# LorenzoNajt/FlipComplexityEmpirical

Measured on AMD Instinct MI355X. Metric: flip proposals/sec (node) 40x40 grid k=2, 1/2/4/8 MI355X; % LDS/HBM roofline, higher is better.
Workload: dtype int8

## Files before the change

### flipcomplexityempirical_amd/csrc/fc_device.h

```cpp
#pragma once
#include <hip/hip_runtime.h>
#include <stdint.h>

#include <type_traits>

#include "fc_internal.h"
#include "fc_philox.h"
#include "fc_ring.h"

namespace fc {
namespace dev {

__device__ __forceinline__ void compiler_fence() { asm volatile("" ::: "memory"); }
__device__ __forceinline__ void wave_sync() { asm volatile("s_waitcnt lgkmcnt(0)" ::: "memory"); }

#ifdef FC_PHASE_PROF
#ifdef FC_PHASE_SYNC
#define FC_STAMP(t)                                                    \
    asm volatile("s_waitcnt vmcnt(0) lgkmcnt(0)" ::: "memory");        \
    const int64_t t = (int64_t)__builtin_amdgcn_s_memtime()
#else
#define FC_STAMP(t) const int64_t t = (int64_t)__builtin_amdgcn_s_memtime()
#endif
#define FC_PROF(i, x) \
    do { if (lane == 0) atomicAdd((unsigned long long *)&prof_acc[i], (unsigned long long)(int64_t)(x)); } while (0)
#else
#define FC_STAMP(t)
#define FC_PROF(i, x)
#endif

__device__ __forceinline__ uint64_t bits_below(int n) { return n >= 64 ? ~0ull : ((1ull << n) - 1ull); }
__device__ __forceinline__ uint64_t lane_range(int lo, int hi) { return bits_below(hi) & ~bits_below(lo); }

__device__ __forceinline__ int rl32(int x, int lane) { return __builtin_amdgcn_readlane(x, lane); }
__device__ __forceinline__ uint32_t rlu(uint32_t x, int lane) { return (uint32_t)__builtin_amdgcn_readlane((int)x, lane); }

__device__ __forceinline__ int64_t rl64(int64_t x, int lane) {
    const uint32_t lo = rlu((uint32_t)x, lane), hi = rlu((uint32_t)((uint64_t)x >> 32), lane);
    return (int64_t)(((uint64_t)hi << 32) | lo);
}
template <typename... T>
__device__ __forceinline__ void wave_sum64_all(T &...x) {
#pragma unroll
    for (int off = 32; off >= 1; off >>= 1) ((x += __shfl_xor((long long)x, off)), ...);
}
__device__ __forceinline__ int64_t wave_sum64(int64_t x) {
    wave_sum64_all(x);
    return x;
}

template <int CTRL>
__device__ __forceinline__ int32_t dpp_pair(int32_t x) {
    return __builtin_amdgcn_update_dpp(x, x, CTRL, 0xf, 0xf, false);
}
constexpr int kQuadSwap1 = 0xB1;
constexpr int kQuadSwap2 = 0x4E;
constexpr int kRowHalfMirror = 0x141;
constexpr int kRowMirror = 0x140;

__device__ __forceinline__ int32_t row0_sum(int32_t x) {
    x += dpp_pair<kQuadSwap1>(x);
    x += dpp_pair<kQuadSwap2>(x);
    x += dpp_pair<kRowHalfMirror>(x);
    x += dpp_pair<kRowMirror>(x);
    return rl32(x, 0);
}
__device__ __forceinline__ int32_t min_lanes32(int32_t x) {
    x = min(x, dpp_pair<kQuadSwap1>(x));
    x = min(x, dpp_pair<kQuadSwap2>(x));
    x = min(x, dpp_pair<kRowHalfMirror>(x));
    x = min(x, dpp_pair<kRowMirror>(x));
    return min(rl32(x, 0), rl32(x, 16));
}

__device__ __forceinline__ int count_below(uint64_t m) {
    return (int)__builtin_amdgcn_mbcnt_hi((uint32_t)(m >> 32), __builtin_amdgcn_mbcnt_lo((uint32_t)m, 0u));
}

template <int CTRL>
__device__ __forceinline__ int dpp_mov(int x) {
    return __builtin_amdgcn_update_dpp(0, x, CTRL, 0xf, 0xf, false);
}

__device__ __forceinline__ int wave_scan_incl(int x) {
    x += dpp_mov<0x111>(x);
    x += dpp_mov<0x112>(x);
    x += dpp_mov<0x114>(x);
    x += dpp_mov<0x118>(x);
    x += __builtin_amdgcn_update_dpp(0, x, 0x142, 0xa, 0xf, false);
    x += __builtin_amdgcn_update_dpp(0, x, 0x143, 0xc, 0xf, false);
    return x;
}

__device__ __forceinline__ int select_bit64(uint64_t x, int r) {
    uint32_t y = (uint32_t)x;
    int pos = 0, c = __popc(y);
    if (r >= c) { r -= c; y = (uint32_t)(x >> 32); pos = 32; }
    c = __popc(y & 0xffffu);
    if (r >= c) { r -= c; y >>= 16; pos += 16; }
    c = __popc(y & 0xffu);
    if (r >= c) { r -= c; y >>= 8; pos += 8; }
    c = __popc(y & 0xfu);
    if (r >= c) { r -= c; y >>= 4; pos += 4; }
    c = __popc(y & 0x3u);
    if (r >= c) { r -= c; y >>= 2; pos += 2; }
    return pos + (r >= (int)(y & 1u) ? 1 : 0);
}

__device__ __forceinline__ int kth_set_bit(uint64_t x, int k) {
    for (int i = 1; i < k; ++i) x &= x - 1;
    return __builtin_ctzll(x);
}

template <int RMAX>
__device__ __forceinline__ int ring_entry(const uint32_t (&ring)[RMAX / 2], int i) {
    return (int)((ring[i >> 1] >> (16 * (i & 1))) & 0xffffu);
}

template <int RMAX>
__device__ __forceinline__ int ring_entry_at(const uint32_t (&ring)[RMAX / 2], uint32_t pos) {
    const uint32_t sel = 0x0c0c0100u + (pos & 3u) * 0x0202u;
    uint32_t e = __builtin_amdgcn_perm(ring[1], ring[0], sel);
#pragma unroll
    for (int k = 1; k < RMAX / 4; ++k) {
        const uint32_t q = __builtin_amdgcn_perm(ring[2 * k + 1], ring[2 * k], sel);
        e = ((pos >> 2) == (uint32_t)k) ? q : e;
    }
    return (int)e;
}

using fc::one_run;
using fc::one_run_flat;

__device__ __forceinline__ int deal_chain(const KParams &p, int lane) {
    int cc = 0;
    if (lane == 0) {
        uint32_t hw, xcc;
        asm volatile("s_getreg_b32 %0, hwreg(HW_REG_HW_ID)" : "=s"(hw));
        asm volatile("s_getreg_b32 %0, hwreg(HW_REG_XCC_ID)" : "=s"(xcc));
        const uint32_t key = ((xcc & 7u) << 12) | ((hw >> 4) & 0xfffu);
        const uint32_t slot = atomicAdd(&p.deal[key], 1u);
        const uint32_t C = (uint32_t)p.n_chains;
        for (uint32_t k = 0; k < 4; ++k) {
            const uint32_t q = (slot + k) & 3u;
            const uint32_t lo = q * C / 4u, hi = (q + 1u) * C / 4u;
            const uint32_t i = atomicAdd(&p.deal[kDealKeys + q], 1u);
            if (lo + i < hi) {
                cc = (int)p.order[lo + i];
                break;
            }
        }
    }
    return __builtin_amdgcn_readfirstlane(__shfl(cc, 0));
}

constexpr int kBfsList = 512;
struct BfsScratch {
    uint32_t *lab;
    uint32_t *mm;
    uint32_t *cm;
// ... 443 lines not shown
```

### flipcomplexityempirical_amd/csrc/fc_flip2.hip

```cpp
#include <hip/hip_runtime.h>

#include <cstdlib>
#include <algorithm>
#include <type_traits>

#include "fc_device.h"
#include "fc_internal.h"
#include "fc_philox.h"
#include "fc_tally.h"

namespace fc {

using namespace dev;

#ifndef FC_PRIO_EVERY_LOG2
#define FC_PRIO_EVERY_LOG2 4
#endif
static_assert(sizeof(KParams) % 8 == 0, "flip2_kernel's second argument sits at sizeof(KParams)");
template <bool FULL>
__device__ __forceinline__ PhiloxKeys batch_keys(PhiloxKeys keys) {
    typedef const unsigned char __attribute__((address_space(4))) *KernArg;
    if constexpr (FULL) {
        KernArg ka = (KernArg)__builtin_amdgcn_kernarg_segment_ptr();
        asm volatile("" : "+s"(ka));
// ... 196 lines not shown
    int prio = 0;
    if (lane == 0) {
        misc[3] = 0;
        misc[4] = (uint64_t)steps_in;
        if (FULL && p.tl_t0) p.tl_t0[c] = steps_in;
        misc[0] = __builtin_amdgcn_s_memrealtime();
        const float eta0 = p.eta ? (float)p.eta[p.eta_parity ^ 1] * (float)p.n_steps * (1.0f / 1024.0f) : 0.0f;
        misc[1] = (uint64_t)__float_as_uint(eta0);
    }
    compiler_fence();
    while (rem > 0) {
        const bool every = ((prio += 4) & (((1 << FC_PRIO_EVERY_LOG2) - 1) << 2)) == 0;
        if (every) cnt_fold();
        if (every && p.prio_nb[0] > 0) {
            const int done = (int)p.n_steps - rem;
            const float eta = __uint_as_float((uint32_t)misc[1]);
            int lv;
            if (eta > 0.0f && done * 16 >= (int)p.n_steps) {
                const float pr = (float)(__builtin_amdgcn_s_memrealtime() - misc[0]) * (float)p.n_steps / ((float)done * eta);
                lv = (pr > p.prio_th[0]) + (pr > p.prio_th[1]) + (pr > p.prio_th[2]);
            } else {
                lv = (nb < p.prio_nb[0]) + (nb < p.prio_nb[1]) + (nb < p.prio_nb[2]);
            }
            if (lv != (prio & 3)) {
                prio = (prio & ~3) | lv;
                switch (lv) {
                    case 0: __builtin_amdgcn_s_setprio(0); break;
                    case 1: __builtin_amdgcn_s_setprio(1); break;
                    case 2: __builtin_amdgcn_s_setprio(2); break;
                    default: __builtin_amdgcn_s_setprio(3); break;
                }
            }
        }
        FC_STAMP(t_a);
        FC_PROF(5, 1);
        if (draw >= draw_cap) {
            stuck = 1;
            break;
        }
        const uint64_t room = draw_cap - draw;
        int nh = 0;
        int gen = 0;
        int rv[kRV];
        auto rv_off = [&](int j, int l) { return BAND ? 64 * j + l : 4 * l + j - (int)(draw & 3u); };
        if constexpr (!BAND) {
            const int s0 = (int)(draw & 3u);
            const int wcap = 64 * NSUB < 4 * kWave - s0 ? 64 * NSUB : 4 * kWave - s0;
            const int win = (uint64_t)wcap < room ? wcap : (int)room;
            const uint64_t q = (draw >> 2) + (uint64_t)lane;
            uint32_t nw[4];
            if (XTRA && p.tape) {
#pragma unroll
                for (int j = 0; j < 4; ++j) {
                    const int off = 4 * lane + j - s0;
                    const bool inr = off >= 0 && off < win;
                    nw[j] = p.tape[((size_t)c * (size_t)p.tape_draws + (inr ? draw + (uint64_t)off : draw)) * 6];
                }
            } else {
                const PhiloxKeys pk = batch_keys<FULL>(keys);
                const Words4 w = philox4x32_10_keys((uint32_t)q, (uint32_t)(q >> 32), chain_gid, 3u, pk);
                nw[0] = w.x0;
                nw[1] = w.x1;
                nw[2] = w.x2;
                nw[3] = w.x3;
            }
            int vdj[4];
            uint32_t okm = 0u, hb = 0u;
#pragma unroll
            for (int j = 0; j < 4; ++j) {
                const int off = 4 * lane + j - s0;
                const uint64_t m = (uint64_t)nw[j] * (uint64_t)(uint32_t)n;
                vdj[j] = (int)(m >> 32);
                const bool ok = (off >= 0) & (off < win) & ((uint32_t)m >= p.lemire_thresh);
                okm |= (uint32_t)ok << j;
                hb |= (uint32_t)(ok & (fcnt[vdj[j]] != 0)) << j;
            }
            const int hc = __popc(hb);
            const int incl = wave_scan_incl(hc);
            const int excl = incl - hc;
            const int tot = rl32(incl, kWave - 1);
            gen = win;
            int lim = 4 * kWave;
            if (tot > 64) {
                const int L = __builtin_ctzll(__ballot(incl >= 64));
                const uint32_t hbL = rlu(hb, L);
                const int k = 64 - rl32(excl, L);
                uint32_t mk = hbL;
                for (int i = 1; i < k; ++i) mk &= mk - 1u;
                const int jj = __builtin_ctz(mk);
                lim = 4 * L + jj - s0 + 1;
                gen = lim;
            }
            uint32_t *const ssink = slot + 256 + lane;
#pragma unroll
            for (int j = 0; j < 4; ++j) {
                const int off = 4 * lane + j - s0;
                const int sp = excl + __popc(hb & ((1u << j) - 1u));
                const bool hit = (hb >> j) & 1u;
                const bool put = hit & (sp < 64);
                *(put ? slot + sp : ssink) = (uint32_t)vdj[j];
                *(put ? slot + 192 + sp : ssink) = (uint32_t)off;
                rv[j] = (((okm >> j) & 1u) & !hit & (off < lim)) ? (vdj[j] | (sp << 16)) : -1;
            }
            nh = tot;
        } else {
            int bpre = 0x7fffffff;
            {
                const int cw = lane < p.words ? (int)__popcll(sb[lane]) : 0;
                const int inc = wave_scan_incl(cw);
                if (lane < p.words) bpre = inc - cw;
            }
#pragma unroll
            for (int r = 0; r < NSUB; ++r) {
                rv[r] = -1;
                if ((r > 0 && nh >= p.hit_stop) || nh >= 64 || (uint64_t)gen >= room) continue;
                const int off = gen + lane;
                const bool inrange = (uint64_t)off < room;
                const uint64_t dr = draw + (uint64_t)off;
                const Words4 w = philox4x32_10((uint32_t)dr, (uint32_t)(dr >> 32), chain_gid, 0u, p.seed_lo, p.seed_hi);
                const uint64_t m = (uint64_t)w.x0 * (uint64_t)nS;
                const int idx = (int)(m >> 32);
                const bool okd = inrange && (uint32_t)m >= thrS;
                int bw = 0, bb = 0;
                for (int st2 = p.band_step0; st2 >= 1; st2 >>= 1) {
                    const int cand = bw + st2;
                    const int pc = __builtin_amdgcn_ds_bpermute(cand << 2, bpre);
                    if (pc <= idx) {
                        bw = cand;
                        bb = pc;
                    }
                }
                const int vd = 64 * bw + select_bit64(sb[bw], idx - bb);
                const bool hitd = okd & (fcnt[vd] != 0);
                const uint64_t hm = __ballot(hitd);
                const int sp = nh + count_below(hm);
                if (hitd && sp < 64) {
                    slot[sp] = (uint32_t)vd;
                    slot[64 + sp] = w.x1;
                    slot[128 + sp] = w.x2;
                    slot[192 + sp] = (uint32_t)off;
                }
                const int cnt = __popcll(hm);
                int used = kWave;
                if (nh + cnt > 64) {
                    used = kth_set_bit(hm, 64 - nh) + 1;
                    gen += used;
                } else {
                    gen = (uint64_t)(gen + 64) < room ? gen + 64 : (int)room;
                }
                rv[r] = (okd & !hitd & (lane < used)) ? (vd | (sp << 16)) : rv[r];
                nh += cnt;
            }
        }
        const int ns = nh < 64 ? nh : 64;
        compiler_fence();
        FC_STAMP(t_b);
        FC_PROF(1, t_b - t_a);

        const bool has = lane < ns;
        const int off_r = (int)slot[192 + lane], v_r = (int)slot[lane];
        int off_l = has ? off_r : gen;
        const uint64_t d = draw + (uint64_t)off_l;
        int v = has ? v_r : 0;
        uint32_t w1, w2;
        if constexpr (BAND) {
            w1 = slot[64 + lane];
            w2 = slot[128 + lane];
// ... 65 lines not shown
        bool rebuild = false;
        const int cut0 = cut, nb0 = nb;
        const int64_t steps0 = FULL ? steps_in + ((int)p.n_steps - rem) : 0;
        const int last_flip0 = last_flip;
        const int a_last0 = FULL && last_flip0 >= 0 ? (int)a[last_flip0] : 0;
        int cut_after = 0, nb_after = 0;
        auto dp_of = [&]() { return av == 0 ? -pv : pv; };
        auto dg_of = [&]() { return (st & LF_GAM) ? (av == 0 ? -1 : 1) : 0; };

        auto reeval = [&](int from, int vfx, uint32_t eqx) {
            FC_STAMP(t_re0);
            compiler_fence();
            if (has && lane >= from) {
                const uint32_t lkl = slot[256 + lane];
                const uint32_t w1r = (!FULL && !BAND) ? w1 : slot[64 + lane], w2r = (!FULL && !BAND) ? w2 : slot[128 + lane];
                if (vfx < 0) {
                    av = a[v];
                    uint32_t i1 = 0;
                    int ad[RMAX];
#pragma unroll
                    for (int i = 0; i < RMAX; ++i) ad[i] = a[cell[i]];
#pragma unroll
                    for (int i = 0; i < RMAX; ++i) asm volatile("" : "+v"(ad[i]));
#pragma unroll
                    for (int i = 0; i < RMAX; ++i) i1 |= (uint32_t)ad[i] << i;
                    inA = av ? i1 : ~i1;
                } else {
                    const bool self = v == vfx;
                    av = self ? 1 - av : av;
                    inA = (self ? ~inA : inA) ^ eqx;
                }
                const uint32_t nbA = inA & nbr;
                tmask = nbr & ~inA;
                nA = __popc(nbA);
                delta = nA - __popc(tmask);
                const uint64_t th = T[delta + RMAX];
                const uint32_t lnk = lkl & 0xffffu, L2 = lkl >> 16;
                const uint32_t fl = (1u << L2) - 1u;
                inA &= fl;
                const uint32_t rot = L2 ? (((inA >> 1) | (inA << (L2 - 1))) & fl) : 0u;
                const uint32_t lk = inA & rot & lnk;
                const bool sl = one_run_flat(nbA, fl & ~lk, fl);
                const uint32_t vlink = (L2 >= 2) ? ((inA & (inA >> (L2 - 1)) & 1u) << (L2 - 1)) : 0u;
                const bool sc = one_run_flat(nbA, fl & ~(lk | vlink), fl);
                const bool ac = mant53(w1r, w2r) < th;
                st = (st & (LF_EXACT | LF_GAM | LF_HAS | LF_FRZ)) | (tmask != 0u ? LF_HIT : 0u) | (ac ? LF_ACC : 0u) |
                     (sl ? LF_SLIN : 0u) | (sc ? LF_SCYC : 0u);
            }
            compiler_fence();
            FC_STAMP(t_re1);
            FC_PROF(16, t_re1 - t_re0);
            FC_PROF(17, 1);
        };

        auto run_bfs = [&](int f) -> bool {
            const uint32_t nbrAf = rlu(inA & nbr, f);
            int my_target = -1, start = -1;
#pragma unroll
            for (int k2 = 0; k2 < RMAX / 2; ++k2) {
                const uint32_t wrd = rlu(rec.ring[k2], f);
                if ((lane >> 1) == k2) my_target = (int)((wrd >> (16 * (lane & 1))) & 0xffffu);
                if (start < 0 && ((nbrAf >> (2 * k2)) & 1u)) start = (int)(wrd & 0xffffu);
                if (start < 0 && ((nbrAf >> (2 * k2 + 1)) & 1u)) start = (int)(wrd >> 16);
            }
            if (!(lane < RMAX && ((nbrAf >> lane) & 1u))) my_target = -1;
            int64_t lv = 0;
            const bool res = wave_bfs_single<RMAX>(G, a, bs, lane, rl32(v, f), rl32(av, f), my_target, start, lv);
            if (lane == 0) {
                atomicAdd((unsigned long long *)&scp->bfs_calls, 1ull);
                atomicAdd((unsigned long long *)&scp->bfs_levels, (unsigned long long)lv);
            }
            return res;
        };

        while (pos < end) {
            FC_PROF(6, 1);
            FC_STAMP(t_it0);
#ifdef FC_PHASE_PROF
            if (first_it) FC_PROF(27, t_it0 - t_c);
            first_it = false;
#endif
            asm volatile("" : "+v"(st), "+v"(inA), "+v"(tmask), "+v"(nbr), "+v"(delta), "+v"(nA), "+v"(av), "+v"(pv),
                         "+v"(v), "+v"(off_l));
            const bool hit = (st & LF_HIT) != 0, acc = (st & LF_ACC) != 0, s_lin = (st & LF_SLIN) != 0,
                       s_cyc = (st & LF_SCYC) != 0, exact = SEARCH ? (st & LF_EXACT) != 0 : true,
                       gam = (st & LF_GAM) != 0, has = (st & LF_HAS) != 0;
            const bool prop = hit & (lane >= pos) & (lane < end);
            const bool bd = SEARCH && (st & ST_BD) != 0, br = SEARCH && (st & ST_BR) != 0, nz = nA != 0;
            const bool okT = bd ? br : (nz & s_lin);
            const bool okN = bd ? br : (nz & ((exact & gam) ? s_cyc : s_lin));
            const bool known = bd | !nz | exact | s_lin;
            const bool ok = ((av ? ng0 : ng1) > 0) ? okT : okN;
            const int pa = av ? pops1 : pops0, pb = av ? pops0 : pops1;
            const bool popok = (pa - pv >= pop_lo) & (pb + pv <= pop_hi);
            bool valid = prop & known & ok & popok;
            bool acc_now = acc;
            bool inv_contig = !ok;
            if constexpr (XTRA) {
                if (p.variant) {
                    const int gm = gam ? 1 : 0;
                    const bool b_ok = ((av ? ng1 : ng0) - gm > 0) && ((av ? ng0 : ng1) + gm > 0);
                    const bool f_ok = !(st & LF_FRZ);
                    auto pass = [&](uint32_t M) {
                        return (!(M & FC_CON_CONTIG) || ok) && (!(M & FC_CON_POP) || popok) &&
                               (!(M & FC_CON_BOUNDARY) || b_ok) && (!(M & FC_CON_FIXED) || f_ok);
                    };
                    valid = prop && known && pass(p.con_valid);
                    inv_contig = (p.con_valid & FC_CON_CONTIG) && !ok;
                    bool au = acc;
                    if (p.accept == FC_ACCEPT_UNIFORM) {
                        au = true;
                    } else if (p.accept == FC_ACCEPT_ANNEAL) {
                        int dnb_l = nA == 0 ? -1 : 0;
#pragma unroll
                        for (int i = 0; i < RMAX; ++i) {
                            const int oc = fcnt[cell[i]];
                            const bool nb_i = (nbr >> i) & 1u;
                            dnb_l += nb_i ? (int)(((inA >> i) & 1u) && oc == 0) - (int)(((tmask >> i) & 1u) && oc == 1) : 0;
                        }
                        const double bw = __longlong_as_double((long long)T[delta + RMAX]);
                        const double bound = bw * ((double)(nb + dnb_l) / (double)nb);
                        au = (double)mant53(w1, w2) * 0x1p-53 < bound;
                    }
                    acc_now = pass(p.con_accept) && au;
                }
            }
            const uint64_t C0 = __ballot(valid && acc_now);
            FC_STAMP(t_it1);
            FC_PROF(8, t_it1 - t_it0);
            if (__popcll(C0) >= p.par_min) {
                FC_PROF(12, 1);
                const bool cand0 = valid && acc;
                const int dp_l = dp_of(), dg_l = dg_of();
                const int x0 = cand0 ? dp_l : 0;
                const int P = wave_scan_incl(x0) - x0;
                const int Gp = count_below(__ballot(cand0 && dg_l > 0)) - count_below(__ballot(cand0 && dg_l < 0));
                const bool ok1 = ((av ? ng0 + Gp : ng1 - Gp) > 0) ? okT : okN;
                const int q0 = pops0 + P, q1 = pops1 - P;
                const bool valid1 = prop & known & ok1 & ((av ? q1 : q0) - pv >= pop_lo) &
                                    ((av ? q0 : q1) + pv <= pop_hi);
                const bool cand1 = valid1 && acc;
                const uint64_t MM = __ballot(prop && cand1 != cand0);
                const uint64_t UU = __ballot(prop && !known);
                int sg = end;
                if (MM) sg = min(sg, __builtin_ctzll(MM) + 1);
                const int u = UU ? __builtin_ctzll(UU) : kWave;
                if (u < sg) sg = u;
                uint64_t VAL = __ballot(valid1) & lane_range(pos, sg);
                bool last_step = false;
                if (__popcll(VAL) >= rem) {
                    sg = kth_set_bit(VAL, rem) + 1;
                    VAL &= bits_below(sg);
                    last_step = true;
                }
                const uint64_t K = __ballot(cand1) & lane_range(pos, sg);
                int x = kWave;
                bool stale_seg = false;
                NbrCells nc;
                const RingCells<RMAX> rc{cell};
                uint32_t nm = 0u;
                auto nbr_bits = [&]() { return LIST ? nm : nbr; };
                auto ina_bits = [&]() { return LIST ? nm >> 16 : inA; };
                auto marks_put = [&](const auto &cl, uint32_t wm) {
                    constexpr int N = std::decay_t<decltype(cl)>::N;
#pragma unroll
                    for (int i = 0; i < N; ++i) FC_ST((wm >> i) & 1u, nmark[cl[i]], lane);
                };
                auto marks_get = [&](const auto &cl, uint32_t &gt, uint32_t &lt) {
                    constexpr int N = std::decay_t<decltype(cl)>::N;
                    int mn[N];
#pragma unroll
                    for (int i = 0; i < N; ++i) mn[i] = nmark[cl[i]];
                    gt = 0u;
                    lt = 0u;
#pragma unroll
                    for (int i = 0; i < N; ++i) {
                        gt |= (uint32_t)(mn[i] > lane) << i;
                        lt |= (uint32_t)(mn[i] < lane) << i;
                    }
                };
                if (K) {
                    const bool inK = (K >> lane) & 1ull;
                    if constexpr (LIST) {
                        uint32_t npos = (uint32_t)(rec.meta >> kMetaPosShift);
                        asm volatile("" : "+v"(npos));
                        nm = (1u << min((int)__popc(nbr), 4)) - 1u;
                        uint32_t e[4];
#pragma unroll
                        for (int i = 0; i < 4; ++i) {
                            const uint32_t ps = (npos >> (4 * i)) & 15u;
                            e[i] = (uint32_t)ring_entry_at<RMAX>(rec.ring, ps);
                            nm |= ((inA >> ps) & 1u) << (16 + i);
                        }
                        nc.w[0] = e[0] | (e[1] << 16);
                        nc.w[1] = e[2] | (e[3] << 16);
                        asm volatile("" : "+v"(nc.w[0]), "+v"(nc.w[1]));
                    }
                    st |= inK ? LF_WROTE : 0u;
                    bool need = inK;
                    int ms = 0xff, mk[kRV];
                    uint32_t gtm = 0xffffu, ltm = 0u;
                    for (;;) {
                        FC_PROF(21, 1);
                        FC_ST(need && ms > lane, smark[v], lane);
                        const uint32_t wm = need ? (nbr_bits() & gtm) : 0u;
                        if constexpr (LIST) marks_put(nc, wm);
                        else marks_put(rc, wm);
                        compiler_fence();
                        ms = smark[v];
#pragma unroll
                        for (int r = 0; r < kRV; ++r) mk[r] = nmark[rv[r] < 0 ? 0 : (rv[r] & 0xffff)];
                        if constexpr (LIST) marks_get(nc, gtm, ltm);
                        else marks_get(rc, gtm, ltm);
                        const bool again = (ms > lane) | ((nbr_bits() & gtm) != 0u);
                        need = need & again;
                        if (!__any(need)) break;
                    }
                    FC_STAMP(t_mk);
                    FC_PROF(18, t_mk - t_it1);
                    bool conf = (ms < lane) | (inK & ((nbr_bits() & ltm) != 0u));
#pragma unroll
                    for (int i = 0; i < RMAX; ++i) conf |= (int)smark[cell[i]] < lane;
                    conf &= has;
                    const uint64_t XX = __ballot(conf && lane > pos && lane < end);
                    if (XX) {
                        x = __builtin_ctzll(XX);
                        stale_seg = true;
                        FC_PROF(13, 1);
                    }
                    int t = trunc_off;
#pragma unroll
                    for (int r = 0; r < kRV; ++r) {
                        const bool tr = (rv[r] >= 0) & (mk[r] < x) & (mk[r] < (rv[r] >> 16));
                        const uint64_t TR = __ballot(tr);
                        if (TR) t = min(t, rv_off(r, __builtin_ctzll(TR)));
                    }
                    if (t < trunc_off) {
                        trunc_off = t;
                        const int e2 = __popcll(__ballot(has && off_l < t));
                        if (e2 < x) x = e2;
                        if (e2 < end) end = e2;
                        FC_PROF(14, 1);
                    }
                }
                FC_STAMP(t_cf);
                FC_PROF(19, t_cf - t_it1);
                int ce = min(sg, x);
                bool seg_out = false;
                if constexpr (BAND) {
                    const uint64_t K0 = K & bits_below(ce);
                    if (K0) {
                        bool out = false;
                        if ((K0 >> lane) & 1ull) {
#pragma unroll
                            for (int i = 0; i < RMAX; ++i) {
                                const int u = cell[i];
                                const uint32_t oc = fcnt[u];
                                const uint64_t swd = sb[u >> 6];
                                out |= ((nbr & inA) >> i & 1u) && oc == 0u && !((swd >> (u & 63)) & 1ull);
                            }
                        }
                        const uint64_t IV = __ballot(out);
                        if (IV) {
                            ce = __builtin_ctzll(IV) + 1;
                            seg_out = true;
                            if (ce < sg) last_step = false;
                        }
                    }
                }
                if (x < sg) last_step = false;
                if (prop && lane < ce) st |= valid1 ? (cand1 ? (ST_VS | ST_AC) : ST_VS) : (ok1 ? ST_IP : ST_IC);
                rem -= __popcll(VAL & bits_below(ce));
                const uint64_t AP = K & bits_below(ce);
                if (AP) {
                    FC_PROF(7, __popcll(AP));
                    const bool me = (AP >> lane) & 1ull;
                    int dnb = 0;
                    const uint32_t nbm = me ? nbr_bits() : 0u;
                    auto counts = [&](const auto &cl) {
                        constexpr int N = std::decay_t<decltype(cl)>::N;
                        int oldc[N];
#pragma unroll
                        for (int i = 0; i < N; ++i) oldc[i] = fcnt[cl[i]];
                        compiler_fence();
#pragma unroll
                        for (int i = 0; i < N; ++i) {
                            const int nw = oldc[i] + 2 * (int)((ina_bits() >> i) & 1u) - 1;
                            const uint32_t nb_i = (nbm >> i) & 1u;
                            FC_ST(nb_i, fcnt[cl[i]], nw);
                            dnb += (min(nw, 1) - min(oldc[i], 1)) & -(int)nb_i;
                        }
                    };
                    if constexpr (LIST) counts(nc);
                    else counts(rc);
                    FC_ST(me, *(uint8_t *)&a[v], 1 - av);
                    FC_ST(me, fcnt[v], nA);
                    const int pkd = me ? ((delta + 32) | ((dnb + 32) << 16)) : 0;
                    const int S = wave_scan_incl(pkd);
                    const int cntA = count_below(AP) + 1;
                    cut_after = me ? cut + (S & 0xffff) - 32 * cntA : cut_after;
                    nb_after = me ? nb + (S >> 16) - 32 * cntA : nb_after;
                    const int L = 63 - __builtin_clzll(AP);
                    cut = rl32(cut_after, L);
                    nb = rl32(nb_after, L);
                    const int dP = rl32(P + dp_l, L), dG = rl32(Gp + dg_l, L);
                    pops0 += dP;
                    pops1 -= dP;
                    ng0 += dG;
                    ng1 -= dG;
                    last_flip = rl32(v, L);
                    compiler_fence();
                }
                if (st & LF_WROTE) {
                    smark[v] = 0xff;
                    if constexpr (LIST) {
#pragma unroll
                        for (int i = 0; i < 4; ++i) nmark[nc[i]] = 0xff;
                    } else {
#pragma unroll
                        for (int i = 0; i < RMAX; ++i) nmark[cell[i]] = 0xff;
                    }
                    st &= ~LF_WROTE;
                }
                FC_STAMP(t_sg1);
                FC_PROF(11, t_sg1 - t_it1);
                pos = ce;
                if (BAND && seg_out) rebuild = true;
                if (last_step) {
                    end = pos;
                    target_hit = true;
                    break;
                }
                if (BAND && seg_out) {
                    end = pos;
                    trunc_off = rl32(off_l, pos - 1) + 1;
                    break;
                }
                if (pos >= end) break;
                if (stale_seg && AP) {
                    reeval(pos, -1, 0u);
                    FC_STAMP(t_sg2);
                    FC_PROF(29, t_sg2 - t_sg1);
                    continue;
                }
                if (SEARCH && u == pos) {
                    const bool res = run_bfs(u);
                    if (lane == u) st |= ST_BD | (res ? ST_BR : 0u);
                }
                FC_STAMP(t_sg3);
                FC_PROF(29, t_sg3 - t_sg1);
                continue;
            }
            const uint64_t VAL = __ballot(valid);
            const uint64_t EV = C0 | __ballot(prop && !known);
            const int f = EV ? __builtin_ctzll(EV) : end;
            const uint64_t segv = VAL & bits_below(f);
            const int nvalid = __popcll(segv);
            const uint32_t bits = valid ? ST_VS : (inv_contig ? ST_IC : ST_IP);
            if (nvalid >= rem) {
                const int e = kth_set_bit(segv, rem);
                st |= (prop & (lane <= e)) ? bits : 0u;
                rem = 0;
                end = e + 1;
                target_hit = true;
                break;
            }
            st |= (prop & (lane < f)) ? bits : 0u;
            rem -= nvalid;
            pos = f;
            if (f >= end) {
                FC_STAMP(t_fx);
                FC_PROF(25, t_fx - t_it1);
                break;
            }
            if (SEARCH && !((VAL >> f) & 1ull)) {
                const bool res = run_bfs(f);
                if (lane == f) st |= ST_BD | (res ? ST_BR : 0u);
                continue;
            }
            FC_PROF(7, 1);
            FC_STAMP(t_ap0);
            FC_PROF(9, t_ap0 - t_it1);
            const int vf = rl32(v, f), Af = rl32(av, f), pvf = rl32(pv, f), df = rl32(delta, f);
            const uint32_t inAf = rlu(inA, f), nbrf = rlu(nbr, f), tmf = rlu(tmask, f);
            const bool gamf = rl32((int)gam, f) != 0;
            uint32_t rw[RMAX / 2];
#pragma unroll
            for (int k2 = 0; k2 < RMAX / 2; ++k2) rw[k2] = rlu(rec.ring[k2], f);
            uint32_t sel = rw[0];
#pragma unroll
            for (int k2 = 1; k2 < RMAX / 2; ++k2) sel = ((lane >> 1) == k2) ? rw[k2] : sel;
            const int my_e = (int)((sel >> (16 * (lane & 1))) & 0xffffu);
            const bool is_nbr = lane < RMAX && ((nbrf >> lane) & 1u);
            const int dlt = (int)((inAf >> lane) & 1u) - (int)((tmf >> lane) & 1u);
            const int old = fcnt[my_e];
            FC_ST(is_nbr, fcnt[my_e], old + dlt);
            const bool enter = is_nbr & (dlt > 0) & (old == 0);
            const bool leave = is_nbr & (dlt < 0) & (old == 1);
            bool outS = false;
            if constexpr (BAND) {
                const uint64_t swd = sb[my_e >> 6];
                outS = enter && !((swd >> (my_e & 63)) & 1ull);
            }
            if (lane == 0) {
                a[vf] = (int8_t)(1 - Af);
                fcnt[vf] = (uint8_t)__popc(nbrf & inAf);
            }
            uint32_t eqm = 0;
#pragma unroll
            for (int i = 0; i < RMAX; ++i) eqm |= (uint32_t)(cell[i] == vf) << i;
            const bool stale = has & ((v == vf) | (eqm != 0u));
            const uint64_t aff = __ballot(stale && lane > f && lane < end);
            if (aff) FC_PROF(13, 1);
            uint64_t ent = __ballot(enter);
            const int dnb = __popcll(ent) - __popcll(__ballot(leave));
            if (ent) {
                int t_na = trunc_off;
                int fr[kRV];
#pragma unroll
                for (int r = 0; r < kRV; ++r) fr[r] = fcnt[rv[r] < 0 ? 0 : (rv[r] & 0xffff)];
#pragma unroll
                for (int r = 0; r < kRV; ++r) {
                    const bool tr = (rv[r] >= 0) & ((rv[r] >> 16) > f) & (fr[r] != 0);
                    const uint64_t m2 = __ballot(tr);
                    if (m2) t_na = min(t_na, rv_off(r, __builtin_ctzll(m2)));
                }
                if (t_na < trunc_off) {
                    trunc_off = t_na;
                    const int e2 = __popcll(__ballot(has && off_l < t_na));
                    if (e2 < end) end = e2;
                    FC_PROF(14, 1);
                }
            }
            if (Af == 0) {
                pops0 -= pvf;
                pops1 += pvf;
            } else {
                pops1 -= pvf;
                pops0 += pvf;
            }
            if (gamf) {
                const int dg = Af == 0 ? -1 : 1;
                ng0 += dg;
                ng1 -= dg;
            }
            cut += df;
            nb += dnb;
            --rem;
            last_flip = vf;
            const bool me_f = lane == f;
            st |= me_f ? (ST_VS | ST_AC) : 0u;
            cut_after = me_f ? cut : cut_after;
            nb_after = me_f ? nb : nb_after;
            compiler_fence();
            FC_STAMP(t_ap1);
            FC_PROF(10, t_ap1 - t_ap0);
            pos = f + 1;
            const bool f_out = BAND && __ballot(outS) != 0ull;
            if (f_out) rebuild = true;
            if (rem == 0) {
                end = pos;
                target_hit = true;
                break;
            }
            if (f_out) {
                end = pos;
                trunc_off = rl32(off_l, f) + 1;
                break;
            }
            if (aff && pos < end) reeval(pos, vf, eqm);
            FC_STAMP(t_ap2);
            FC_PROF(30, t_ap2 - t_ap1);
        }
        compiler_fence();
        FC_STAMP(t_d);
        FC_PROF(3, t_d - t_c);

        FC_PROF(15, (end == ns && !target_hit && trunc_off == gen) ? 1 : 0);
        const bool done = lane < end;
        const bool is_acc = (st & ST_AC) != 0;
        const bool proposed = (st & LF_HIT) && done;
        n_acc += __popcll(__ballot(is_acc));
        n_ic += __popcll(__ballot((st & ST_IC) != 0));
        n_ip += __popcll(__ballot((st & ST_IP) != 0));
        const uint64_t ACCM = __ballot(is_acc);
        const uint64_t VSM = __ballot((st & ST_VS) != 0);
        int ln = lane;
        asm volatile("" : "+v"(ln));
        const uint64_t later_acc = ACCM & ~bits_below(ln + 1);
        const int next_acc = later_acc ? __builtin_ctzll(later_acc) : end;
        const int run_len = is_acc ? 1 + __popcll(VSM & lane_range(ln + 1, next_acc)) : 0;
        const int first_acc = ACCM ? __builtin_ctzll(ACCM) : end;
        const int r0 = __popcll(VSM & bits_below(first_acc));
        int64_t my_wait = 0;
        if (XTRA && want_wait && !defer && is_acc) {
            Words4 g;
            if (XTRA && p.tape) {
                const uint32_t *t = p.tape + ((size_t)c * (size_t)p.tape_draws + d) * 6;
                g = Words4{t[4], t[5], 0u, 0u};
            } else {
                g = philox4x32_10((uint32_t)d, (uint32_t)(d >> 32), chain_gid, 1u, p.seed_lo, p.seed_hi);
            }
            my_wait = geom_wait_of(g.x0, g.x1, p.log1mp[nb_after]);
        }
        if (!defer) {
            const int cr = cut_after * run_len, br = nb_after * run_len;
            acc_cut += cr;
            acc_cut2 += (int64_t)cr * cut_after;
            acc_nb += br;
            acc_nb2 += (int64_t)br * nb_after;
            acc_wait += my_wait * run_len;
        }
        if (lane == 0 && r0 && (!defer || qn == 0)) {
            acc_cut += (int64_t)cut0 * r0;
            acc_cut2 += (int64_t)cut0 * cut0 * r0;
            acc_nb += (int64_t)nb0 * r0;
            acc_nb2 += (int64_t)nb0 * nb0 * r0;
            acc_wait += wait_cur * r0;
        }
        const int64_t t_acc = FULL ? steps0 + __popcll(VSM & bits_below(ln + 1)) : 0;
        if constexpr (FULL) {
            if (lane == 0 && r0 && (!defer || qn == 0) && (p.diag & (FC_DIAG_HIST | FC_DIAG_FLIPS))) {
                const uint32_t qv0 = (last_flip0 >= 0 ? (uint32_t)last_flip0 : 0xffffu) | ((uint32_t)(a_last0 & 1) << 16);
                const int64_t lbase = (int64_t)misc[3];
                if (p.tl && lbase < p.tl_cap) {
                    ((uint4 *)p.tl)[(size_t)c * (size_t)p.tl_cap + (size_t)lbase] =
                        tally_pack(steps0 - (int64_t)misc[4], r0, qv0, (uint32_t)cut0, (uint32_t)nb0 | 0x80000000u);
                    misc[3] = (uint64_t)(lbase + 1);
                } else {
                    tally_apply<RMAX>(p, c, steps0, r0, qv0, (uint32_t)cut0, (uint32_t)nb0 | 0x80000000u, p.labels[0],
                                      p.labels[1]);
                }
            }
        }
        if (defer) {
            if (lane == 0 && r0 && qn > 0) q_run[qn - 1] += (uint32_t)r0;
            const int na = __popcll(ACCM);
            if (na) {
                if (qn > 0 && qn + na > p.wait_q) wait_flush();
                const int qi = qn + count_below(ACCM);
                if (is_acc) {
                    q_d[qi] = d;
                    q_nb[qi] = (uint32_t)nb_after;
                    q_run[qi] = (uint32_t)run_len;
                    q_c[qi] = (uint32_t)cut_after | ((uint32_t)(1 - av) << 31);
                    if constexpr (FULL) {
                        q_v[qi] = (uint32_t)v | ((inA & nbr) << 16);
                        if (qi == 0) misc[2] = (uint64_t)t_acc;
                    }
                }
                qn += na;
                compiler_fence();
            }
        }
        if constexpr (FULL) {
            if (XTRA && !defer && (p.diag & FC_DIAG_SERIES) && ACCM) {
                const int64_t idx = ev_len + __popcll(ACCM & bits_below(ln));
                if (is_acc && idx < p.ev_cap) {
                    fc_event ev;
                    ev.t = t_acc;
                    ev.v = (uint16_t)v;
                    ev.cut = (uint16_t)cut_after;
                    ev.nb = (uint16_t)nb_after;
                    ev.target = (uint8_t)(1 - av);
                    ev.reserved = 0;
                    p.events[(size_t)c * p.ev_cap + idx] = ev;
                }
                ev_len += __popcll(ACCM);
            }
            if (hit_time < 0 && ACCM) {
                const uint64_t hm = __ballot(is_acc && cut_after >= p.hit_lo && cut_after <= p.hit_hi);
                if (hm) {
                    const int hl = __builtin_ctzll(hm);
                    hit_time = steps0 + __popcll(VSM & bits_below(hl + 1));
                }
            }
            if (XTRA && !defer && (p.diag & FC_DIAG_HIST) && is_acc) {
                atomicAdd((unsigned long long *)&p.cut_hist[(size_t)c * (p.n_edges + 1) + cut_after], (unsigned long long)run_len);
                atomicAdd((unsigned long long *)&p.nb_hist[(size_t)c * (n + 1) + nb_after], (unsigned long long)run_len);
            }
            if (XTRA && !defer && (p.diag & FC_DIAG_FLIPS) && is_acc) {
                int64_t *nf = p.num_flips + (size_t)c * n, *ps = p.part_sum + (size_t)c * n;
                unsigned long long *lf = (unsigned long long *)(p.last_flipped + (size_t)c * n);
                const int64_t lsum = (int64_t)p.labels[0] + (int64_t)p.labels[1];
                const int64_t t_last = t_acc + run_len - 1;
                atomicMax(lf + v, (unsigned long long)t_last);
                atomicAdd((unsigned long long *)(ps + v), (unsigned long long)((lsum - 2 * (int64_t)p.labels[1 - av]) * t_last));
                atomicAdd((unsigned long long *)(nf + v), (unsigned long long)run_len);
            }
            if (XTRA && !defer && (p.diag & FC_DIAG_FLIPS_EXACT) && is_acc) {
                const size_t o = (size_t)c * n + v;
                const int64_t dl = (int64_t)p.labels[1 - av] - (int64_t)p.labels[av];
                atomicAdd((unsigned long long *)(p.flip_count + o), 1ull);
                atomicAdd((unsigned long long *)(p.occ_acc + o), (unsigned long long)(-dl * t_acc));
                atomicMax((unsigned long long *)(p.last_accept + o), (unsigned long long)t_acc);
            }
            if (XTRA && !defer && (p.diag & FC_DIAG_EDGES) && is_acc) {
                int64_t *ea = p.edge_acc + (size_t)c * p.n_edges;
                for (int i = 0; i < RMAX; ++i) {
                    if (!((nbr >> i) & 1u)) continue;
                    const int e = p.ring_eid[(size_t)v * RMAX + i];
                    if ((inA >> i) & 1u) {
                        atomicAdd((unsigned long long *)(ea + e), (unsigned long long)(-t_acc));
                    } else if ((tmask >> i) & 1u) {
                        atomicAdd((unsigned long long *)(ea + e), (unsigned long long)t_acc);
                    }
                }
            }
            if (trace_on) {
                const uint64_t PM = __ballot(proposed);
                const uint64_t mine = ACCM & bits_below(ln + 1);
                const int src = mine ? 63 - __builtin_clzll(mine) : 0;
                const int c_j = __shfl(cut_after, src), n_j = __shfl(nb_after, src);
                const long long w_j = __shfl((long long)my_wait, src);
                const int64_t idx = trace_len + __popcll(PM & bits_below(ln));
                if (proposed && idx < p.trace_cap) {
                    fc_record &rr = p.trace[(size_t)c * p.trace_cap + idx];
                    const bool valid = (st & ST_VS) != 0;
                    rr.draw = (int64_t)d;
                    rr.v = v;
                    rr.flags = (valid ? (1 | (is_acc ? 2 : 0)) : ((st & ST_IC) ? 4 : 8)) | ((1 - av) << 8);
                    rr.cut = mine ? c_j : cut0;
                    rr.nb = mine ? n_j : nb0;
                    rr.wait = valid ? (mine ? (int64_t)w_j : wait_cur) : 0;
                }
                trace_len += __popcll(PM);
            }
        }
        if (!defer && ACCM) wait_cur = rl64(my_wait, 63 - __builtin_clzll(ACCM));
        int consumed;
        if (target_hit) {
            consumed = rl32(off_l, end - 1) + 1;
        } else {
            consumed = end < ns ? rl32(off_l, end) : gen;
            if (trunc_off < consumed) consumed = trunc_off;
        }
        draw += (uint64_t)consumed;
        if constexpr (BAND) {
            if (rebuild) {
                FC_STAMP(t_rb0);
                band_rebuild();
                FC_STAMP(t_rb1);
                FC_PROF(22, 1);
                FC_PROF(23, t_rb1 - t_rb0);
            }
        }
        FC_PROF(24, ns);
        compiler_fence();
        FC_STAMP(t_e);
        FC_PROF(4, t_e - t_d);
    }
    if (defer && qn > 0) wait_flush();
    FC_STAMP(t_loop1);
    FC_PROF(0, t_loop1 - t_loop0);
    if (p.ctime && lane == 0) p.ctime[c] = (uint32_t)min(draw - scp->draw, (uint64_t)0xffffffffu);
    if (p.eta && rem == 0 && lane == 0) {
        const uint64_t el = __builtin_amdgcn_s_memrealtime() - misc[0];
        atomicMax(&p.eta[p.eta_parity], (uint32_t)min(el * 1024ull / (uint64_t)max((int)p.n_steps, 1), 0xffffffffull));
    }
#ifdef FC_PHASE_PROF
    wave_sync();
    if (p.prof && lane == 0)
        for (int i = 0; i < kProfSlots; ++i) p.prof[(size_t)c * kProfSlots + i] = prof_acc[i];
#endif

    {
        uint4 *ga = (uint4 *)(p.assign + (size_t)c * npad);
        uint4 *gf = (uint4 *)(p.fcnt + (size_t)c * npad);
        for (int i = lane; i < npad / 16; i += kWave) {
            ga[i] = ((const uint4 *)a)[i];
            gf[i] = ((const uint4 *)fcnt)[i];
        }
        if (BAND && lane < p.words) p.sbits[(size_t)c * p.words + lane] = sb[lane];
    }
    cnt_fold();
    const int taken = (int)p.n_steps - rem;
    const int64_t cnt_acc = rl64(cnt64, 0), cnt_ic = rl64(cnt64, 1), cnt_ip = rl64(cnt64, 2);
    const int64_t cnt_prop = (int64_t)taken + cnt_ic + cnt_ip;
    wave_sum64_all(acc_cut, acc_nb, acc_wait, acc_cut2, acc_nb2);
    if (FULL && p.tl_len && lane == 0) p.tl_len[c] = (int64_t)misc[3];
    if (lane == 0) {
        scp->draw = draw;
        scp->steps = steps_in + taken;
        scp->proposals += cnt_prop;
        scp->accepted += cnt_acc;
        scp->inv_contig += cnt_ic;
        scp->inv_pop += cnt_ip;
        if (FULL) {
            scp->trace_len = trace_len;
            scp->ev_len = ev_len;
            scp->hit_time = hit_time;
        }
        scp->sum_cut += acc_cut;
// ... 59 lines not shown
```

Baseline: 22.31 billion.

## Compute flip validity predicates as wave-wide ballot masks in scalar registers

Replaces per-lane boolean predicate logic in the flip proposal loop with 64-bit ballot masks combined with scalar bitwise ops, using inverse ballot to recover per-lane bools only where needed. The aim is to move the validity, acceptance and conflict logic onto the scalar unit and to cut redundant __ballot calls and VALU compare/select chains. It adds more ballot instructions per predicate and inverse-ballot conversions, and it subtly changes masks such as HAS, rv[r]>=0 and the gamma handling, which risks semantic drift.

New measurement: 23.83 billion (median of 6 runs). 1.07x the previous value.

```diff
diff --git a/flipcomplexityempirical_amd/csrc/fc_device.h b/flipcomplexityempirical_amd/csrc/fc_device.h
--- a/flipcomplexityempirical_amd/csrc/fc_device.h
+++ b/flipcomplexityempirical_amd/csrc/fc_device.h
@@ -76,6 +76,9 @@
 __device__ __forceinline__ int count_below(uint64_t m) {
     return (int)__builtin_amdgcn_mbcnt_hi((uint32_t)(m >> 32), __builtin_amdgcn_mbcnt_lo((uint32_t)m, 0u));
 }
+
+__device__ __forceinline__ uint64_t vote(bool p) { return __builtin_amdgcn_ballot_w64(p); }
+__device__ __forceinline__ bool lanes(uint64_t m) { return __builtin_amdgcn_inverse_ballot_w64(m); }
 
 template <int CTRL>
 __device__ __forceinline__ int dpp_mov(int x) {
diff --git a/flipcomplexityempirical_amd/csrc/fc_flip2.hip b/flipcomplexityempirical_amd/csrc/fc_flip2.hip
--- a/flipcomplexityempirical_amd/csrc/fc_flip2.hip
+++ b/flipcomplexityempirical_amd/csrc/fc_flip2.hip
@@ -302,7 +302,7 @@
             gen = win;
             int lim = 4 * kWave;
             if (tot > 64) {
-                const int L = __builtin_ctzll(__ballot(incl >= 64));
+                const int L = __builtin_ctzll(vote(incl >= 64));
                 const uint32_t hbL = rlu(hb, L);
                 const int k = 64 - rl32(excl, L);
                 uint32_t mk = hbL;
@@ -534,22 +534,28 @@
 #endif
             asm volatile("" : "+v"(st), "+v"(inA), "+v"(tmask), "+v"(nbr), "+v"(delta), "+v"(nA), "+v"(av), "+v"(pv),
                          "+v"(v), "+v"(off_l));
-            const bool hit = (st & LF_HIT) != 0, acc = (st & LF_ACC) != 0, s_lin = (st & LF_SLIN) != 0,
-                       s_cyc = (st & LF_SCYC) != 0, exact = SEARCH ? (st & LF_EXACT) != 0 : true,
-                       gam = (st & LF_GAM) != 0, has = (st & LF_HAS) != 0;
-            const bool prop = hit & (lane >= pos) & (lane < end);
-            const bool bd = SEARCH && (st & ST_BD) != 0, br = SEARCH && (st & ST_BR) != 0, nz = nA != 0;
-            const bool okT = bd ? br : (nz & s_lin);
-            const bool okN = bd ? br : (nz & ((exact & gam) ? s_cyc : s_lin));
-            const bool known = bd | !nz | exact | s_lin;
-            const bool ok = ((av ? ng0 : ng1) > 0) ? okT : okN;
+            const uint64_t HIT = vote((st & LF_HIT) != 0u), ACC = vote((st & LF_ACC) != 0u),
+                           SLIN = vote((st & LF_SLIN) != 0u), SCYC = vote((st & LF_SCYC) != 0u),
+                           GAM = vote((st & LF_GAM) != 0u);
+            const uint64_t EXACT = SEARCH ? vote((st & LF_EXACT) != 0u) : ~0ull;
+            const uint64_t HAS = bits_below(ns);
+            const uint64_t PROP = HIT & lane_range(pos, end);
+            const uint64_t BD = SEARCH ? vote((st & ST_BD) != 0u) : 0ull, BR = SEARCH ? vote((st & ST_BR) != 0u) : 0ull;
+            const uint64_t NZ = vote(nA != 0);
+            const uint64_t OKT = (BD & BR) | (~BD & NZ & SLIN);
+            const uint64_t OKN = (BD & BR) | (~BD & NZ & ((EXACT & GAM & SCYC) | (~(EXACT & GAM) & SLIN)));
+            const uint64_t KNOWN = BD | ~NZ | EXACT | SLIN;
+            const uint64_t OT = vote((av ? ng0 : ng1) > 0);
+            const uint64_t OK = (OT & OKT) | (~OT & OKN);
             const int pa = av ? pops1 : pops0, pb = av ? pops0 : pops1;
-            const bool popok = (pa - pv >= pop_lo) & (pb + pv <= pop_hi);
-            bool valid = prop & known & ok & popok;
-            bool acc_now = acc;
-            bool inv_contig = !ok;
+            const uint64_t POPOK = vote(pa - pv >= pop_lo) & vote(pb + pv <= pop_hi);
+            uint64_t VALID = PROP & KNOWN & OK & POPOK;
+            uint64_t ACC_NOW = ACC;
+            uint64_t INV_CONTIG = ~OK;
             if constexpr (XTRA) {
                 if (p.variant) {
+                    const bool gam = lanes(GAM), ok = lanes(OK), popok = lanes(POPOK), prop = lanes(PROP),
+                               known = lanes(KNOWN), acc = lanes(ACC);
                     const int gm = gam ? 1 : 0;
                     const bool b_ok = ((av ? ng1 : ng0) - gm > 0) && ((av ? ng0 : ng1) + gm > 0);
                     const bool f_ok = !(st & LF_FRZ);
@@ -557,8 +563,8 @@
                         return (!(M & FC_CON_CONTIG) || ok) && (!(M & FC_CON_POP) || popok) &&
                                (!(M & FC_CON_BOUNDARY) || b_ok) && (!(M & FC_CON_FIXED) || f_ok);
                     };
-                    valid = prop && known && pass(p.con_valid);
-                    inv_contig = (p.con_valid & FC_CON_CONTIG) && !ok;
+                    VALID = vote(prop && known && pass(p.con_valid));
+                    INV_CONTIG = (p.con_valid & FC_CON_CONTIG) ? ~OK : 0ull;
                     bool au = acc;
                     if (p.accept == FC_ACCEPT_UNIFORM) {
                         au = true;
@@ -574,38 +580,40 @@
                         const double bound = bw * ((double)(nb + dnb_l) / (double)nb);
                         au = (double)mant53(w1, w2) * 0x1p-53 < bound;
                     }
-                    acc_now = pass(p.con_accept) && au;
-                }
-            }
-            const uint64_t C0 = __ballot(valid && acc_now);
+                    ACC_NOW = vote(pass(p.con_accept) && au);
+                }
+            }
+            const uint64_t C0 = VALID & ACC_NOW;
             FC_STAMP(t_it1);
             FC_PROF(8, t_it1 - t_it0);
             if (__popcll(C0) >= p.par_min) {
                 FC_PROF(12, 1);
-                const bool cand0 = valid && acc;
+                const uint64_t CAND0 = VALID & ACC;
                 const int dp_l = dp_of(), dg_l = dg_of();
-                const int x0 = cand0 ? dp_l : 0;
+                const int x0 = lanes(CAND0) ? dp_l : 0;
                 const int P = wave_scan_incl(x0) - x0;
-                const int Gp = count_below(__ballot(cand0 && dg_l > 0)) - count_below(__ballot(cand0 && dg_l < 0));
-                const bool ok1 = ((av ? ng0 + Gp : ng1 - Gp) > 0) ? okT : okN;
+                const uint64_t AV = vote(av != 0);
+                const int Gp = count_below(CAND0 & GAM & AV) - count_below(CAND0 & GAM & ~AV);
+                const uint64_t OT1 = vote((av ? ng0 + Gp : ng1 - Gp) > 0);
+                const uint64_t OK1 = (OT1 & OKT) | (~OT1 & OKN);
                 const int q0 = pops0 + P, q1 = pops1 - P;
-                const bool valid1 = prop & known & ok1 & ((av ? q1 : q0) - pv >= pop_lo) &
-                                    ((av ? q0 : q1) + pv <= pop_hi);
-                const bool cand1 = valid1 && acc;
-                const uint64_t MM = __ballot(prop && cand1 != cand0);
-                const uint64_t UU = __ballot(prop && !known);
+                const uint64_t VALID1 = PROP & KNOWN & OK1 & vote((av ? q1 : q0) - pv >= pop_lo) &
+                                        vote((av ? q0 : q1) + pv <= pop_hi);
+                const uint64_t CAND1 = VALID1 & ACC;
+                const uint64_t MM = PROP & (CAND1 ^ CAND0);
+                const uint64_t UU = PROP & ~KNOWN;
                 int sg = end;
                 if (MM) sg = min(sg, __builtin_ctzll(MM) + 1);
                 const int u = UU ? __builtin_ctzll(UU) : kWave;
                 if (u < sg) sg = u;
-                uint64_t VAL = __ballot(valid1) & lane_range(pos, sg);
+                uint64_t VAL = VALID1 & lane_range(pos, sg);
                 bool last_step = false;
                 if (__popcll(VAL) >= rem) {
                     sg = kth_set_bit(VAL, rem) + 1;
                     VAL &= bits_below(sg);
                     last_step = true;
                 }
-                const uint64_t K = __ballot(cand1) & lane_range(pos, sg);
+                const uint64_t K = CAND1 & lane_range(pos, sg);
                 int x = kWave;
                 bool stale_seg = false;
                 NbrCells nc;
@@ -632,7 +640,7 @@
                     }
                 };
                 if (K) {
-                    const bool inK = (K >> lane) & 1ull;
+                    const bool inK = lanes(K);
                     if constexpr (LIST) {
                         uint32_t npos = (uint32_t)(rec.meta >> kMetaPosShift);
                         asm volatile("" : "+v"(npos));
@@ -650,6 +658,7 @@
                     }
                     st |= inK ? LF_WROTE : 0u;
                     bool need = inK;
+                    uint64_t NEED = K;
                     int ms = 0xff, mk[kRV];
                     uint32_t gtm = 0xffffu, ltm = 0u;
                     for (;;) {
@@ -664,17 +673,16 @@
                         for (int r = 0; r < kRV; ++r) mk[r] = nmark[rv[r] < 0 ? 0 : (rv[r] & 0xffff)];
                         if constexpr (LIST) marks_get(nc, gtm, ltm);
                         else marks_get(rc, gtm, ltm);
-                        const bool again = (ms > lane) | ((nbr_bits() & gtm) != 0u);
-                        need = need & again;
-                        if (!__any(need)) break;
+                        NEED &= vote(ms > lane) | vote((nbr_bits() & gtm) != 0u);
+                        need = lanes(NEED);
+                        if (!NEED) break;
                     }
                     FC_STAMP(t_mk);
                     FC_PROF(18, t_mk - t_it1);
-                    bool conf = (ms < lane) | (inK & ((nbr_bits() & ltm) != 0u));
-#pragma unroll
-                    for (int i = 0; i < RMAX; ++i) conf |= (int)smark[cell[i]] < lane;
-                    conf &= has;
-                    const uint64_t XX = __ballot(conf && lane > pos && lane < end);
+                    uint64_t CONF = vote(ms < lane) | (K & vote((nbr_bits() & ltm) != 0u));
+#pragma unroll
+                    for (int i = 0; i < RMAX; ++i) CONF |= vote((int)smark[cell[i]] < lane);
+                    const uint64_t XX = CONF & HAS & lane_range(pos + 1, end);
                     if (XX) {
                         x = __builtin_ctzll(XX);
                         stale_seg = true;
@@ -683,13 +691,12 @@
                     int t = trunc_off;
 #pragma unroll
                     for (int r = 0; r < kRV; ++r) {
-                        const bool tr = (rv[r] >= 0) & (mk[r] < x) & (mk[r] < (rv[r] >> 16));
-                        const uint64_t TR = __ballot(tr);
+                        const uint64_t TR = vote(mk[r] < x) & vote(mk[r] < (rv[r] >> 16));
                         if (TR) t = min(t, rv_off(r, __builtin_ctzll(TR)));
                     }
                     if (t < trunc_off) {
                         trunc_off = t;
-                        const int e2 = __popcll(__ballot(has && off_l < t));
+                        const int e2 = __popcll(HAS & vote(off_l < t));
                         if (e2 < x) x = e2;
                         if (e2 < end) end = e2;
                         FC_PROF(14, 1);
@@ -721,12 +728,13 @@
                     }
                 }
                 if (x < sg) last_step = false;
-                if (prop && lane < ce) st |= valid1 ? (cand1 ? (ST_VS | ST_AC) : ST_VS) : (ok1 ? ST_IP : ST_IC);
+                if (lanes(PROP & bits_below(ce)))
+                    st |= lanes(VALID1) ? (lanes(CAND1) ? (ST_VS | ST_AC) : ST_VS) : (lanes(OK1) ? ST_IP : ST_IC);
                 rem -= __popcll(VAL & bits_below(ce));
                 const uint64_t AP = K & bits_below(ce);
                 if (AP) {
                     FC_PROF(7, __popcll(AP));
-                    const bool me = (AP >> lane) & 1ull;
+                    const bool me = lanes(AP);
                     int dnb = 0;
                     const uint32_t nbm = me ? nbr_bits() : 0u;
                     auto counts = [&](const auto &cl) {
@@ -803,21 +811,21 @@
                 FC_PROF(29, t_sg3 - t_sg1);
                 continue;
             }
-            const uint64_t VAL = __ballot(valid);
-            const uint64_t EV = C0 | __ballot(prop && !known);
+            const uint64_t VAL = VALID;
+            const uint64_t EV = C0 | (PROP & ~KNOWN);
             const int f = EV ? __builtin_ctzll(EV) : end;
             const uint64_t segv = VAL & bits_below(f);
             const int nvalid = __popcll(segv);
-            const uint32_t bits = valid ? ST_VS : (inv_contig ? ST_IC : ST_IP);
+            const uint32_t bits = lanes(VALID) ? ST_VS : (lanes(INV_CONTIG) ? ST_IC : ST_IP);
             if (nvalid >= rem) {
                 const int e = kth_set_bit(segv, rem);
-                st |= (prop & (lane <= e)) ? bits : 0u;
+                st |= lanes(PROP & bits_below(e + 1)) ? bits : 0u;
                 rem = 0;
                 end = e + 1;
                 target_hit = true;
                 break;
             }
-            st |= (prop & (lane < f)) ? bits : 0u;
+            st |= lanes(PROP & bits_below(f)) ? bits : 0u;
             rem -= nvalid;
             pos = f;
             if (f >= end) {
@@ -835,7 +843,7 @@
             FC_PROF(9, t_ap0 - t_it1);
             const int vf = rl32(v, f), Af = rl32(av, f), pvf = rl32(pv, f), df = rl32(delta, f);
             const uint32_t inAf = rlu(inA, f), nbrf = rlu(nbr, f), tmf = rlu(tmask, f);
-            const bool gamf = rl32((int)gam, f) != 0;
+            const bool gamf = (GAM >> f) & 1ull;
             uint32_t rw[RMAX / 2];
 #pragma unroll
             for (int k2 = 0; k2 < RMAX / 2; ++k2) rw[k2] = rlu(rec.ring[k2], f);
@@ -843,16 +851,16 @@
 #pragma unroll
             for (int k2 = 1; k2 < RMAX / 2; ++k2) sel = ((lane >> 1) == k2) ? rw[k2] : sel;
             const int my_e = (int)((sel >> (16 * (lane & 1))) & 0xffffu);
-            const bool is_nbr = lane < RMAX && ((nbrf >> lane) & 1u);
-            const int dlt = (int)((inAf >> lane) & 1u) - (int)((tmf >> lane) & 1u);
+            const uint64_t NBRF = nbrf & ((1u << RMAX) - 1u), INAF = NBRF & inAf, TMF = NBRF & tmf;
+            const bool is_nbr = lanes(NBRF);
+            const int dlt = lanes(INAF) ? 1 : (lanes(TMF) ? -1 : 0);
             const int old = fcnt[my_e];
             FC_ST(is_nbr, fcnt[my_e], old + dlt);
-            const bool enter = is_nbr & (dlt > 0) & (old == 0);
-            const bool leave = is_nbr & (dlt < 0) & (old == 1);
-            bool outS = false;
+            const uint64_t ENTER = INAF & vote(old == 0), LEAVE = TMF & vote(old == 1);
+            uint64_t OUTS = 0ull;
             if constexpr (BAND) {
                 const uint64_t swd = sb[my_e >> 6];
-                outS = enter && !((swd >> (my_e & 63)) & 1ull);
+                OUTS = ENTER & vote(((swd >> (my_e & 63)) & 1ull) == 0ull);
             }
             if (lane == 0) {
                 a[vf] = (int8_t)(1 - Af);
@@ -861,11 +869,10 @@
             uint32_t eqm = 0;
 #pragma unroll
             for (int i = 0; i < RMAX; ++i) eqm |= (uint32_t)(cell[i] == vf) << i;
-            const bool stale = has & ((v == vf) | (eqm != 0u));
-            const uint64_t aff = __ballot(stale && lane > f && lane < end);
+            const uint64_t aff = (vote(v == vf) | vote(eqm != 0u)) & HAS & lane_range(f + 1, end);
             if (aff) FC_PROF(13, 1);
-            uint64_t ent = __ballot(enter);
-            const int dnb = __popcll(ent) - __popcll(__ballot(leave));
+            const uint64_t ent = ENTER;
+            const int dnb = __popcll(ent) - __popcll(LEAVE);
             if (ent) {
                 int t_na = trunc_off;
                 int fr[kRV];
@@ -873,13 +880,12 @@
                 for (int r = 0; r < kRV; ++r) fr[r] = fcnt[rv[r] < 0 ? 0 : (rv[r] & 0xffff)];
 #pragma unroll
                 for (int r = 0; r < kRV; ++r) {
-                    const bool tr = (rv[r] >= 0) & ((rv[r] >> 16) > f) & (fr[r] != 0);
-                    const uint64_t m2 = __ballot(tr);
+                    const uint64_t m2 = vote((rv[r] >> 16) > f) & vote(fr[r] != 0);
                     if (m2) t_na = min(t_na, rv_off(r, __builtin_ctzll(m2)));
                 }
                 if (t_na < trunc_off) {
                     trunc_off = t_na;
-                    const int e2 = __popcll(__ballot(has && off_l < t_na));
+                    const int e2 = __popcll(HAS & vote(off_l < t_na));
                     if (e2 < end) end = e2;
                     FC_PROF(14, 1);
                 }
@@ -908,7 +914,7 @@
             FC_STAMP(t_ap1);
             FC_PROF(10, t_ap1 - t_ap0);
             pos = f + 1;
-            const bool f_out = BAND && __ballot(outS) != 0ull;
+            const bool f_out = BAND && OUTS != 0ull;
             if (f_out) rebuild = true;
             if (rem == 0) {
                 end = pos;
@@ -929,14 +935,12 @@
         FC_PROF(3, t_d - t_c);
 
         FC_PROF(15, (end == ns && !target_hit && trunc_off == gen) ? 1 : 0);
-        const bool done = lane < end;
         const bool is_acc = (st & ST_AC) != 0;
-        const bool proposed = (st & LF_HIT) && done;
-        n_acc += __popcll(__ballot(is_acc));
-        n_ic += __popcll(__ballot((st & ST_IC) != 0));
-        n_ip += __popcll(__ballot((st & ST_IP) != 0));
-        const uint64_t ACCM = __ballot(is_acc);
-        const uint64_t VSM = __ballot((st & ST_VS) != 0);
+        const uint64_t ACCM = vote((st & ST_AC) != 0u);
+        const uint64_t VSM = vote((st & ST_VS) != 0u);
+        n_acc += __popcll(ACCM);
+        n_ic += __popcll(vote((st & ST_IC) != 0u));
+        n_ip += __popcll(vote((st & ST_IP) != 0u));
         int ln = lane;
         asm volatile("" : "+v"(ln));
         const uint64_t later_acc = ACCM & ~bits_below(ln + 1);
@@ -1021,7 +1025,7 @@
                 ev_len += __popcll(ACCM);
             }
             if (hit_time < 0 && ACCM) {
-                const uint64_t hm = __ballot(is_acc && cut_after >= p.hit_lo && cut_after <= p.hit_hi);
+                const uint64_t hm = ACCM & vote(cut_after >= p.hit_lo) & vote(cut_after <= p.hit_hi);
                 if (hm) {
                     const int hl = __builtin_ctzll(hm);
                     hit_time = steps0 + __popcll(VSM & bits_below(hl + 1));
@@ -1060,7 +1064,8 @@
                 }
             }
             if (trace_on) {
-                const uint64_t PM = __ballot(proposed);
+                const uint64_t PM = vote((st & LF_HIT) != 0u) & bits_below(end);
+                const bool proposed = lanes(PM);
                 const uint64_t mine = ACCM & bits_below(ln + 1);
                 const int src = mine ? 63 - __builtin_clzll(mine) : 0;
                 const int c_j = __shfl(cut_after, src), n_j = __shfl(nb_after, src);
```
